# HydrogenSulfate/LFT

Measured on AMD Instinct MI355X. Metric: LF patches/sec (5x5 angRes, 32x32 LR, 4xSR), higher is better.
Workload: dtype bf16; 1 GPU; LFT 5x5 angRes 4xSR inference, batch=4 per GPU, 32x32 LR patches; global_batch=4, parallelism=dp1 (independent shards), streams_per_gpu=1, hip_graph=True, steps_in_flight=2

## Files before the change

### lft_amd/csrc/lft_api.hip

```cpp
#include "../../include/lft_hip.h"
#include "../../include/lft_hip_test.h"
#include <hip/hip_runtime.h>
#include <stdint.h>

#include <cstdarg>
#include <cstdio>
#include <cmath>
#include <set>
#include <string>
#include <algorithm>
#include <type_traits>
#include <utility>
#include <vector>

#ifndef LFT_TU
#define LFT_TU 0
#endif

namespace {
#include "lft_kernels_a.cuh"
#include "lft_kernels_b.cuh"
#include "lft_metrics.cuh"
#include "lft_train.cuh"
}
// ... 9 lines not shown

int fail(int code, const char* fmt, ...) {
    va_list ap;
    va_start(ap, fmt);
    vsnprintf(g_err, sizeof(g_err), fmt, ap);
    va_end(ap);
    return code;
}

#define LFT_HIP_OK(expr)                                                                     \
    do {                                                                                     \
        hipError_t e_ = (expr);                                                              \
        if (e_ != hipSuccess) return fail((int)e_, "%s: %s", #expr, hipGetErrorString(e_));   \
    } while (0)
struct Profiler {
    bool on = false;
    hipStream_t st = nullptr;
    std::vector<hipEvent_t> ev;
    std::vector<const char*> names;
};
thread_local Profiler g_prof;
inline const char* prof_name(const char* plain, const char* fmt, ...) {
    if (!g_prof.on) return plain;
    static thread_local std::set<std::string> names;
    char buf[96];
    va_list ap;
    va_start(ap, fmt);
    vsnprintf(buf, sizeof(buf), fmt, ap);
    va_end(ap);
    return names.insert(buf).first->c_str();
}
inline void prof_mark(const char* name) {
    if (!g_prof.on) return;
    hipEvent_t e;
    if (hipEventCreate(&e) != hipSuccess) return;
    (void)hipEventRecord(e, g_prof.st);
    g_prof.ev.push_back(e);
    g_prof.names.push_back(name);
}

#define LFT_LAUNCH_OK(name)                                                                  \
    do {                                                                                     \
        hipError_t e_ = hipGetLastError();                                                   \
        if (e_ != hipSuccess) return fail((int)e_, "launch %s: %s", name, hipGetErrorString(e_)); \
        prof_mark(name);                                                                     \
    } while (0)

constexpr int kLayers = 4;

template <auto... Vs, typename V, typename F> int dispatch(V v, F&& f) {
    int rc = 0;
    if (((v == Vs && ((rc = f(std::integral_constant<decltype(Vs), Vs>{})), true)) || ...)) return rc;
    return fail(LFT_ERR_ARG, "internal: no kernel variant for %d", (int)v);
}
template <int V> using int_c = std::integral_constant<int, V>;
template <typename F> int by_prec(int prec, F&& f) {
    if (prec == LFT_PREC_F32) return f(float{});
    if (prec == LFT_PREC_BF16) return f(bf16_t{});
    return f(f16_t{});
}
inline size_t align256(size_t x) { return (x + 255) & ~(size_t)255; }

struct Dims {
    int B, A, V, h, w, hw, s, gp, gt, nchunk;
    long long ntok;
};

int make_dims(int B, int A, int h, int w, int s, int prec, Dims* d) {
    if (prec != LFT_PREC_F32 && prec != LFT_PREC_BF16 && prec != LFT_PREC_F16)
        return fail(LFT_ERR_ARG, "prec must be LFT_PREC_F32, LFT_PREC_BF16 or LFT_PREC_F16, got %d", prec);
    if (B < 1 || A < 1 || h < 1 || w < 1) return fail(LFT_ERR_SHAPE, "B, A, h, w must be positive (B=%d A=%d h=%d w=%d)", B, A, h, w);
    if (s != 2 && s != 4) return fail(LFT_ERR_SHAPE, "scale factor must be 2 or 4, got %d", s);
    if (A * A > 128) return fail(LFT_ERR_UNSUPPORTED, "angRes %d (A*A=%d views > 128) is not implemented in this build", A, A * A);
    if ((long long)B * A * A * h * w > (1LL << 27)) return fail(LFT_ERR_SHAPE, "too many tokens");
    d->B = B; d->A = A; d->V = A * A; d->h = h; d->w = w; d->hw = h * w; d->s = s;
    d->gp = (s + 2) * (s + 2); d->gt = (d->gp + 31) / 32; d->nchunk = 2 * s * s;
    d->ntok = (long long)B * d->V * d->hw;
    return 0;
}

constexpr int kFragsConv = 72, kFragsAng = 64, kFragsSpa1 = 240, kFragsSpa1NoQ = 208, kFragsSpa2 = 176;
inline int frags_up(const Dims& d) { return d.nchunk * (4 + 2 * d.gt); }

struct PackedLayout {
    size_t conv0_w, ln_ang[kLayers], ln_spa[kLayers], ang_pe, petok[kLayers], spa_pe_img;
    size_t s_conv[3], s_ang[kLayers], s_spa1[kLayers], s_spa2[kLayers], s_up, total;
};

PackedLayout packed_layout(const Dims& d, int prec) {
    const size_t esz = prec == LFT_PREC_F32 ? 4 : 2, fragb = 64 * 8 * esz;
    PackedLayout L;
    size_t o = 0;
    auto take = [&](size_t bytes) { size_t r = o; o = align256(o + bytes); return r; };
    L.conv0_w = take(576 * 4);
    for (int l = 0; l < kLayers; ++l) { L.ln_ang[l] = take(256 * 4); L.ln_spa[l] = take(512 * 4); }
    L.ang_pe = take((size_t)((d.V + 31) / 32) * 2048 * 4);
    for (int l = 0; l < kLayers; ++l) L.petok[l] = take((size_t)((d.hw + 32 * kNwSpa1 - 1) / (32 * kNwSpa1)) * kNwSpa1 * 4096 * esz);
    L.spa_pe_img = take((size_t)d.hw * 64 * esz);
    for (int i = 0; i < 3; ++i) L.s_conv[i] = take(kFragsConv * fragb);
    for (int l = 0; l < kLayers; ++l) {
        L.s_ang[l] = take(kFragsAng * fragb);
        L.s_spa1[l] = take(kFragsSpa1 * fragb);
        L.s_spa2[l] = take(kFragsSpa2 * fragb);
    }
    L.s_up = take((size_t)frags_up(d) * fragb);
    L.total = o;
    return L;
}

struct WorkLayout {
    size_t x0, feat, xa, xb, tok, q, k, v, o, g, status, total;
};
WorkLayout work_layout(const Dims& d, int prec) {
    const size_t esz = prec == LFT_PREC_F32 ? 4 : 2;
    WorkLayout W;
    size_t o = 0;
    auto take = [&](size_t bytes) { size_t r = o; o = align256(o + bytes); return r; };
    const size_t n = (size_t)d.ntok;
    W.x0 = take(n * 64 * esz); W.feat = take(n * 64 * esz); W.xa = take(n * 64 * esz); W.xb = take(n * 64 * esz);
    W.tok = take(n * 128 * esz); W.q = take(n * 128 * esz); W.k = take(n * 128 * esz); W.v = take(n * 128 * esz);
    W.o = take(n * 128 * esz);
    W.g = take(n * d.gp * 4);
    W.status = take(256);
    W.total = o;
    return W;
}

template <typename T> size_t lds_conv64(int w) { return WRing<T, kConv64Chunk, kNwConv>::LDS_BYTES + ConvIn<T, kNwConv>::bytes(w) + kNwConv * TileIO<2, T>::BYTES + kConvZeroRow; }
constexpr size_t kLdsParams = 1024;
template <typename T, int CH = kSpaChunk> size_t lds_spa1(int w) {
    return WRing<T, CH, kNwSpa1>::LDS_BYTES + std::max<size_t>(ConvIn<T, kNwSpa1>::bytes(w), (size_t)kNwSpa1 * TileIO<4, T>::BYTES) + kLdsParams + kConvZeroRow;
}
template <typename T> size_t lds_spa2() { return WRing<T, kSpaChunk, kNwSpa2>::LDS_BYTES + kLdsParams + kNwSpa2 * TileIO<4, T>::BYTES; }
template <typename T> size_t lds_up() { return WRing<T, kUpChunk, kNwUp>::LDS_BYTES + kNwUp * TileIO<2, T>::BYTES; }
template <typename T> size_t lds_ang() { return (size_t)kFragsAng * 1024 * FragInfo<T>::PIECES + kLdsParams + 4 * TileIO<2, T>::BYTES; }
constexpr size_t kMaxLds = 160 * 1024;
template <typename K> int allow_lds(K kernel, size_t bytes, const char* name) {
    if (bytes > kMaxLds) return fail(LFT_ERR_SHAPE, "%s needs %zu B of LDS (> 160 KiB): view width too large for this build", name, bytes);
    if (bytes <= 64 * 1024) return 0;
    struct Done { int dev; const void* fn; size_t bytes; };
    static thread_local std::vector<Done> done;
    const void* fn = reinterpret_cast<const void*>(kernel);
    int dev = 0;
    LFT_HIP_OK(hipGetDevice(&dev));
    for (const auto& d : done)
        if (d.dev == dev && d.fn == fn && d.bytes >= bytes) return 0;
    LFT_HIP_OK(hipFuncSetAttribute(fn, hipFuncAttributeMaxDynamicSharedMemorySize, (int)bytes));
    done.push_back(Done{dev, fn, bytes});
    return 0;
}

template <typename P> P* at(const void* base, size_t off) { return reinterpret_cast<P*>(const_cast<char*>(static_cast<const char*>(base)) + off); }
inline unsigned blocks_for(long long items, int per_block) { return (unsigned)((items + per_block - 1) / per_block); }

PackOp lin_op(const float* src, int row0, int nrows, int ld, int k0, int ksteps, int kmap, float scale, int kmul = 1, int kadd = 0) {
    PackOp p{};
    p.src = src; p.kind = 0; p.row0 = row0; p.nrows = nrows; p.ntiles = (nrows + 31) / 32; p.ld = ld;
    p.kmul = kmul; p.kadd = kadd; p.k0 = k0; p.ksteps = ksteps; p.kmap = kmap; p.scale = scale; p.s = 0; p.frag0 = 0;
    return p;
}
void conv_ops(std::vector<PackOp>& v, const float* w, int nout) {
    for (int tap = 0; tap < 9; ++tap)
        for (int ks = 0; ks < 4; ++ks) v.push_back(lin_op(w, 0, nout, 576, 16 * ks, 1, 0, 1.0f, 9, tap));
}

template <typename T>
int run_pack(std::vector<PackOp>& ops, T* dst, int expect_frags, hipStream_t st) {
    int total = 0;
    size_t i = 0;
    while (i < ops.size()) {
        PackArgs a{};
        int nf = 0;
        while (i < ops.size() && a.nops < LFT_PACK_MAXOPS) {
            a.op[a.nops] = ops[i];
            a.op[a.nops].frag0 = nf;
            nf += ops[i].ntiles * ops[i].ksteps;
            ++a.nops; ++i;
        }
        k_pack<T><<<nf, 64, 0, st>>>(a, dst + (size_t)total * 512);
        LFT_LAUNCH_OK("k_pack");
        total += nf;
    }
    if (total != expect_frags) return fail(LFT_ERR_ARG, "internal: stream has %d fragments, expected %d", total, expect_frags);
    return 0;
}

template <typename T> bool tok_lane_major(const Dims& d) {
    return d.hw % (32 * kNwSpa1) == 0 && (sizeof(T) == 4 || d.w % 32 == 0);
}
template <typename T, bool PE_ONLY>
int launch_spa1(unsigned nwg, const T* in, const T* ws, const float* ln, const T* petok, T* tok, T* q, T* k, T* v, T* pe_out,
                int nimg, const Dims& d, hipStream_t st, unsigned* status) {
    const size_t l16 = lds_spa1<T, 16>(d.w), l8 = lds_spa1<T, 8>(d.w);
    const size_t share = kMaxLds / kSpaOcc;
    const bool use8 = (l16 > share && l8 <= share) || l16 > kMaxLds;
    const bool lm = !PE_ONLY && tok_lane_major<T>(d);
    return dispatch<8, 16>(use8 ? 8 : 16, [&](auto CH) {
        return dispatch<true, false>(lm, [&](auto LM) {
            constexpr bool WQ = !(LM && sizeof(T) == 2);
            const size_t lds = CH == 8 ? l8 : l16;
            if (int rc = allow_lds(k_spa1<T, PE_ONLY, CH, LM, WQ>, lds, "k_spa1")) return rc;
            k_spa1<T, PE_ONLY, CH, LM, WQ><<<nwg, 64 * kNwSpa1, lds, st>>>(in, ws, ln, petok, tok, q, k, v, pe_out, nimg, d.h, d.w, status);
            return 0;
        });
    });
}

template <typename T>
int pack_impl(const float* const* P, void* packed, const Dims& d, int prec, hipStream_t st) {
    const PackedLayout L = packed_layout(d, prec);
    const float kAngScale = 0.35355339059327373f * LFT_LOG2E;
    const float kSpaScale = 0.25f * LFT_LOG2E;
    int rc;
    k_copy_f32<<<3, 256, 0, st>>>(P[0], at<float>(packed, L.conv0_w), 576);
    LFT_LAUNCH_OK("k_copy_f32");
    for (int i = 0; i < 3; ++i) {
        std::vector<PackOp> ops;
        conv_ops(ops, P[1 + i], 64);
        if ((rc = run_pack<T>(ops, at<T>(packed, L.s_conv[i]), kFragsConv, st))) return rc;
    }
    k_pe_tables<T><<<blocks_for(std::max<long long>((long long)((d.V + 31) / 32) * 2048, (long long)d.hw * 64), 256), 256, 0, st>>>(
        at<float>(packed, L.ang_pe), at<T>(packed, L.spa_pe_img), d.V, d.h, d.w);
    LFT_LAUNCH_OK("k_pe_tables");
    for (int l = 0; l < kLayers; ++l) {
        const float* const* q = P + 4 + 18 * l;
        float* lnS = at<float>(packed, L.ln_spa[l]);
        float* lnA = at<float>(packed, L.ln_ang[l]);
        const int srcS[4] = {1, 2, 5, 6}, srcA[4] = {10, 11, 14, 15};
        for (int j = 0; j < 4; ++j) {
            k_copy_f32<<<1, 256, 0, st>>>(q[srcS[j]], lnS + 128 * j, 128);
            k_copy_f32<<<1, 256, 0, st>>>(q[srcA[j]], lnA + 64 * j, 64);
        }
        LFT_LAUNCH_OK("k_copy_f32");
        {
            std::vector<PackOp> ops;
            ops.push_back(lin_op(q[12], 0, 64, 64, 0, 4, 1, kAngScale));
            ops.push_back(lin_op(q[12], 64, 64, 64, 0, 4, 1, 1.0f));
            ops.push_back(lin_op(q[12], 128, 64, 64, 0, 4, 1, 1.0f));
            ops.push_back(lin_op(q[13], 0, 64, 64, 0, 4, 1, 1.0f));
            ops.push_back(lin_op(q[16], 0, 128, 64, 0, 4, 1, 1.0f));
            ops.push_back(lin_op(q[17], 0, 64, 128, 0, 8, 1, 1.0f));
            if ((rc = run_pack<T>(ops, at<T>(packed, L.s_ang[l]), kFragsAng, st))) return rc;
        }
        {
            std::vector<PackOp> ops;
            conv_ops(ops, q[0], 128);
            ops.push_back(lin_op(q[3], 256, 128, 128, 0, 8, 1, 1.0f));
            ops.push_back(lin_op(q[3], 128, 128, 128, 0, 8, 1, 1.0f));
            ops.push_back(lin_op(q[3], 0, 128, 128, 0, 8, 1, kSpaScale));
            if ((rc = run_pack<T>(ops, at<T>(packed, L.s_spa1[l]), kFragsSpa1, st))) return rc;
        }
        {
            std::vector<PackOp> ops;
            ops.push_back(lin_op(q[4], 0, 128, 128, 0, 8, (sizeof(T) == 2 && tok_lane_major<T>(d)) ? 1 : 0, 1.0f));
            for (int c = 0; c < 4; ++c) {
                ops.push_back(lin_op(q[7], 64 * c, 64, 128, 0, 8, 1, 1.0f));
                ops.push_back(lin_op(q[8], 0, 128, 256, 64 * c, 4, 1, 1.0f));
            }
            ops.push_back(lin_op(q[9], 0, 64, 128, 0, 8, 1, 1.0f));
            if ((rc = run_pack<T>(ops, at<T>(packed, L.s_spa2[l]), kFragsSpa2, st))) return rc;
        }
        if ((rc = launch_spa1<T, true>((unsigned)((d.hw + 32 * kNwSpa1 - 1) / (32 * kNwSpa1)), at<T>(packed, L.spa_pe_img), at<T>(packed, L.s_spa1[l]), nullptr, nullptr,
                                       nullptr, nullptr, nullptr, nullptr, at<T>(packed, L.petok[l]), 1, d, st, nullptr))) return rc;
        LFT_LAUNCH_OK("k_spa1<pe>");
    }
    {
        std::vector<PackOp> ops;
        for (int c = 0; c < d.nchunk; ++c) {
            ops.push_back(lin_op(P[76], 32 * c, 32, 64, 0, 4, 1, 1.0f));
            PackOp m = lin_op(P[77], 0, d.gp, 0, 32 * c, 2, 1, 1.0f);
            m.kind = 1; m.s = d.s; m.ntiles = d.gt;
            ops.push_back(m);
        }
        if ((rc = run_pack<T>(ops, at<T>(packed, L.s_up), frags_up(d), st))) return rc;
    }
    return 0;
}

void launch_assemble(const float* lr, const float* g, float* out, int B, int A, int h, int w, int s, hipStream_t st, int gld = 0, unsigned* status = nullptr) {
    const dim3 tg((unsigned)((A * w + 7) / 8) * (unsigned)((A * h + 7) / 8) * (unsigned)B);
    if (!gld) gld = (s + 2) * (s + 2);
    if (s == 2) k_assemble_t<2><<<tg, 256, 0, st>>>(lr, g, out, B, A, h, w, gld, status);
    else k_assemble_t<4><<<tg, 256, 0, st>>>(lr, g, out, B, A, h, w, gld, status);
}

template <typename T>
int init_features(const void* packed, const PackedLayout& L, const float* lr, T* x0, T* ta, T* tb, T* feat, const Dims& d, hipStream_t st) {
    const int nimg = d.B * d.V, nwg = nimg * ((d.hw + 32 * kNwConv - 1) / (32 * kNwConv));
    const size_t lds = lds_conv64<T>(d.w);
    int rc;
    if ((rc = allow_lds(k_conv64<T, false>, lds, "k_conv64"))) return rc;
    if ((rc = allow_lds(k_conv64<T, true>, lds, "k_conv64"))) return rc;
    k_conv0<T><<<dim3((unsigned)((d.hw + kConv0Tok - 1) / kConv0Tok), (unsigned)nimg), 256, 0, st>>>(lr, at<float>(packed, L.conv0_w), x0, d.B, d.A, d.h, d.w);
    LFT_LAUNCH_OK("k_conv0");
    k_conv64<T, false><<<nwg, 64 * kNwConv, lds, st>>>(x0, ta, nullptr, at<T>(packed, L.s_conv[0]), nimg, d.h, d.w);
    LFT_LAUNCH_OK("k_conv64");
    k_conv64<T, false><<<nwg, 64 * kNwConv, lds, st>>>(ta, tb, nullptr, at<T>(packed, L.s_conv[1]), nimg, d.h, d.w);
    LFT_LAUNCH_OK("k_conv64");
    k_conv64<T, true><<<nwg, 64 * kNwConv, lds, st>>>(tb, feat, x0, at<T>(packed, L.s_conv[2]), nimg, d.h, d.w);
    LFT_LAUNCH_OK("k_conv64");
    return 0;
}
template <typename T, int CT, int LL>
int ang_multi(const void* packed, const PackedLayout& L, int l, const T* in, T* out, const Dims& d, hipStream_t st, unsigned* status) {
    constexpr bool WLDS = sizeof(T) == 2;
    constexpr int NG = (sizeof(T) == 2 && CT <= 3) ? 2 : 1;
    constexpr size_t FB = 1024 * FragInfo<T>::PIECES;
    const size_t lds = (WLDS ? 64 * FB : 0) + 1024 + (size_t)NG * CT * 8 * FB + (size_t)NG * CT * TileIO<2, T>::BYTES;
    const int npix = d.B * d.hw;
    int rc;
    const unsigned grid = std::min<unsigned>(blocks_for(npix, NG), 256u * (unsigned)std::max<size_t>(1, kMaxLds / lds));
    if ((rc = allow_lds(k_ang_multi<T, CT, WLDS, NG, LL>, lds, "k_ang_multi"))) return rc;
    k_ang_multi<T, CT, WLDS, NG, LL><<<grid, 64 * CT * NG, lds, st>>>(in, out, at<T>(packed, L.s_ang[l]), at<float>(packed, L.ln_ang[l]),
                                                                     at<float>(packed, L.ang_pe), d.V, d.hw, npix, status);
    LFT_LAUNCH_OK("k_ang");
    return 0;
}
template <typename T>
int ang_block(const void* packed, const PackedLayout& L, int l, const T* in, T* out, const Dims& d, hipStream_t st, unsigned* status = nullptr) {
    auto multi = [&](auto CT, auto LL) { return ang_multi<T, CT, LL>(packed, L, l, in, out, d, st, status); };
    if (d.V > 100) return multi(int_c<4>{}, int_c<13>{});
    if (d.V > 96) return multi(int_c<4>{}, int_c<9>{});
    if (d.V > 64) return multi(int_c<3>{}, int_c<9>{});
    if (d.V == 64) return multi(int_c<2>{}, int_c<16>{});
    if (d.V > 32) return multi(int_c<2>{}, int_c<9>{});
    const int npix = d.B * d.hw;
    const size_t lds = lds_ang<T>();
    int rc;
    const unsigned grid = std::min<unsigned>(blocks_for(npix, 4), 256u * (unsigned)std::max<size_t>(1, kMaxLds / lds));
    if ((rc = allow_lds(k_ang<T, 13>, lds, "k_ang"))) return rc;
    k_ang<T, 13><<<grid, 256, lds, st>>>(in, out, at<T>(packed, L.s_ang[l]), at<float>(packed, L.ln_ang[l]),
                                         at<float>(packed, L.ang_pe), d.V, d.hw, npix, status);
    LFT_LAUNCH_OK("k_ang");
    return 0;
}
template <typename T>
int spa_part_a(const void* packed, const PackedLayout& L, int l, const T* in, void* ws, const WorkLayout& W, const Dims& d, hipStream_t st) {
    const int nimg = d.B * d.V, nwg = nimg * ((d.hw + 32 * kNwSpa1 - 1) / (32 * kNwSpa1));
    int rc;
    if ((rc = launch_spa1<T, false>((unsigned)nwg, in, at<T>(packed, L.s_spa1[l]), at<float>(packed, L.ln_spa[l]), at<T>(packed, L.petok[l]),
                                    at<T>(ws, W.tok), at<T>(ws, W.q), at<T>(ws, W.k), at<T>(ws, W.v), nullptr, nimg, d, st, at<unsigned>(ws, W.status)))) return rc;
    LFT_LAUNCH_OK("k_spa1");
    return 0;
}
template <typename F> int with_tail_variant(bool skip, bool tok_lm, bool out_lm, F&& launch) {
    if (out_lm) {
        if (!(skip && tok_lm)) return fail(LFT_ERR_ARG, "internal: lane-major output needs the skip variant and lane-major tokens");
        return launch(std::true_type{}, std::true_type{}, std::true_type{});
    }
    return dispatch<true, false>(skip, [&](auto SK) {
        return dispatch<true, false>(tok_lm, [&](auto LM) { return launch(SK, LM, std::false_type{}); });
    });
}
template <typename T>
int spa_part_b(const void* packed, const PackedLayout& L, int l, const T* skip, T* out, void* ws, const WorkLayout& W,
               const Dims& d, hipStream_t st, bool out_lm = false) {
    const int nimg = d.B * d.V;
    T *tok = at<T>(ws, W.tok), *q = at<T>(ws, W.q), *k = at<T>(ws, W.k), *v = at<T>(ws, W.v), *o = at<T>(ws, W.o);
    const float* ln = at<float>(packed, L.ln_spa[l]);
    const bool lm = tok_lane_major<T>(d);
    int rc;
    if constexpr (sizeof(T) == 2) {
        const unsigned ntile = (unsigned)(nimg * ((d.h + kAttTY - 1) / kAttTY) * ((d.w + kAttTX - 1) / kAttTX));
        if ((rc = with_tail_variant(skip, lm, out_lm, [&](auto SK, auto LM, auto YL) {
                 if (int r = allow_lds(k_spa_b<T, SK, LM, YL>, kSpaBLds, "k_spa_b")) return r;
                 k_spa_b<T, SK, LM, YL><<<ntile, 256, kSpaBLds, st>>>(tok, q, k, v, at<T>(packed, L.s_spa2[l]), ln, skip, out, d.h, d.w,
                                                                      at<unsigned>(ws, W.status), at<T>(packed, L.s_spa1[l]) + (size_t)kFragsSpa1NoQ * 512,
                                                                      at<T>(packed, L.petok[l]));
                 return 0;
             }))) return rc;
        LFT_LAUNCH_OK("k_spa_b");
        return 0;
    } else {
        const unsigned tiles = (unsigned)(((d.w + kWaTX - 1) / kWaTX) * ((d.h + kWaTY - 1) / kWaTY) * nimg);
        if ((rc = allow_lds(k_win_attn_lds<0, true>, kWaLds, "k_win_attn_lds"))) return rc;
        k_win_attn_lds<0, true><<<dim3(tiles, 4), 256, kWaLds, st>>>(reinterpret_cast<const float*>(q), reinterpret_cast<const float*>(k),
                                                                     reinterpret_cast<const float*>(v), reinterpret_cast<float*>(o),
                                                                     nullptr, nullptr, nullptr, nullptr, nullptr, d.h, d.w, 128);
        LFT_LAUNCH_OK("k_spa_attn");
        const unsigned nb = blocks_for(d.ntok, 32 * kNwSpa2);
        if ((rc = with_tail_variant(skip, lm, out_lm, [&](auto SK, auto LM, auto YL) {
                 if (int r = allow_lds(k_spa2<T, SK, LM, YL>, lds_spa2<T>(), "k_spa2")) return r;
                 k_spa2<T, SK, LM, YL><<<nb, 64 * kNwSpa2, lds_spa2<T>(), st>>>(tok, o, at<T>(packed, L.s_spa2[l]), ln, skip, out, d.ntok, at<unsigned>(ws, W.status));
                 return 0;
             }))) return rc;
        LFT_LAUNCH_OK("k_spa2");
        return 0;
    }
}
template <typename T>
int spa_block(const void* packed, const PackedLayout& L, int l, const T* in, const T* skip, T* out, void* ws, const WorkLayout& W,
              const Dims& d, hipStream_t st, bool out_lm = false) {
    int rc;
    if ((rc = spa_part_a<T>(packed, L, l, in, ws, W, d, st))) return rc;
    return spa_part_b<T>(packed, L, l, skip, out, ws, W, d, st, out_lm);
}
template <typename T>
int upsample(const void* packed, const PackedLayout& L, const T* body, const float* lr, float* out, void* ws, const WorkLayout& W,
             const Dims& d, hipStream_t st, bool in_lm = false) {
    float* g = at<float>(ws, W.g);
    const unsigned nb = blocks_for(d.ntok, 32 * kNwUp);
    int rc = dispatch<1, 2>(d.gt, [&](auto GT) {
        return dispatch<true, false>(in_lm, [&](auto LM) {
            if (int r = allow_lds(k_up<T, GT, LM>, lds_up<T>(), "k_up")) return r;
            k_up<T, GT, LM><<<nb, 64 * kNwUp, lds_up<T>(), st>>>(body, at<T>(packed, L.s_up), g, d.ntok, d.nchunk, d.gp);
            return 0;
        });
    });
    if (rc) return rc;
    LFT_LAUNCH_OK("k_up");
    launch_assemble(lr, g, out, d.B, d.A, d.h, d.w, d.s, st, 0, at<unsigned>(ws, W.status));
    LFT_LAUNCH_OK("k_assemble");
    return 0;
}

template <typename T>
int forward_impl(const void* packed, const float* lr, float* out, void* ws, const Dims& d, int prec, hipStream_t st) {
    const PackedLayout L = packed_layout(d, prec);
    const WorkLayout W = work_layout(d, prec);
    T *x0 = at<T>(ws, W.x0), *feat = at<T>(ws, W.feat), *xa = at<T>(ws, W.xa), *xb = at<T>(ws, W.xb);
    int rc;
    if ((rc = init_features<T>(packed, L, lr, x0, xa, xb, feat, d, st))) return rc;
    const T* cur = feat;
    for (int l = 0; l < kLayers; ++l) {
        if ((rc = ang_block<T>(packed, L, l, cur, xa, d, st, at<unsigned>(ws, W.status)))) return rc;
        const bool last = l == kLayers - 1;
        if ((rc = spa_block<T>(packed, L, l, xa, last ? feat : nullptr, xb, ws, W, d, st, last && tok_lane_major<T>(d)))) return rc;
        cur = xb;
    }
    return upsample<T>(packed, L, xb, lr, out, ws, W, d, st, tok_lane_major<T>(d));
}

template <typename T>
int kernel_time_impl(const char* name, const void* packed, void* ws, const Dims& d, int prec, int reps, hipStream_t st, float* ms_out) {
    const PackedLayout L = packed_layout(d, prec);
    const WorkLayout W = work_layout(d, prec);
    T *x0 = at<T>(ws, W.x0), *feat = at<T>(ws, W.feat), *xa = at<T>(ws, W.xa), *xb = at<T>(ws, W.xb);
    const std::string k(name);
    auto once = [&]() -> int {
        if (k == "k_ang") return ang_block<T>(packed, L, 1, xb, xa, d, st, at<unsigned>(ws, W.status));
        if (k == "k_spa1") return spa_part_a<T>(packed, L, 1, xa, ws, W, d, st);
        if (k == "k_spa_b" || k == "k_spa_attn+k_spa2") return spa_part_b<T>(packed, L, 1, nullptr, xb, ws, W, d, st);
        if (k == "k_conv64") {
            const int nimg = d.B * d.V, nwg = nimg * ((d.hw + 32 * kNwConv - 1) / (32 * kNwConv));
            const size_t lds = lds_conv64<T>(d.w);
            int rc;
            if ((rc = allow_lds(k_conv64<T, false>, lds, "k_conv64"))) return rc;
            k_conv64<T, false><<<nwg, 64 * kNwConv, lds, st>>>(x0, feat, nullptr, at<T>(packed, L.s_conv[0]), nimg, d.h, d.w);
            LFT_LAUNCH_OK("k_conv64");
            return 0;
        }
// ... 427 lines not shown
```

### lft_amd/csrc/lft_kernels_b.cuh

```cuda
#pragma once
#include "lft_common.cuh"
#include "lft_kernels_a.cuh"

constexpr int kUpChunk = 8;
constexpr int kSpaChunk = 16;
constexpr int kSpaOcc = 2;
constexpr int kNwSpa1 = 4, kNwSpa2 = 4, kNwUp = 8;
template <typename T, bool PE_ONLY, int CH = kSpaChunk, bool TOKLM = false, bool WITH_Q = true, int NW = kNwSpa1>
__global__ __launch_bounds__(64 * NW, kSpaOcc) void k_spa1(const T* __restrict__ X, const T* __restrict__ ws,
                                              const float* __restrict__ ln, const T* __restrict__ petok,
                                              T* __restrict__ TOK, T* __restrict__ Q, T* __restrict__ K, T* __restrict__ Vv,
                                              T* __restrict__ pe_out, int nimg, int h, int w, unsigned* __restrict__ status) {
    extern __shared__ __attribute__((aligned(16))) char smem[];
    const int lane = threadIdx.x & 63, r = lane & 31, hh = lane >> 5, wave = threadIdx.x >> 6;
    constexpr int TT = 32 * NW;
    const int hw = h * w, tpi = (hw + TT - 1) / TT;
    const int bid = xcd_tile(blockIdx.x, gridDim.x);
    const int im = bid / tpi, p0 = (bid % tpi) * TT;
    const int tl = wave * 32 + r, p = p0 + tl;
    const bool ok = p < hw;
    LFT_STAMP(0);
    typename RawPiece<T>::type pe_raw[16];
    if (!PE_ONLY) load_lane_major_raw<4, T>(petok + (size_t)((p0 >> 5) + wave) * 4096, lane, pe_raw);
    char* lds_in = smem + WRing<T, CH, NW>::LDS_BYTES;
// ... 62 lines not shown
            zero_acc<2>(a);
            linear_ring<2, 8, T>(ring, nf, a);
            if constexpr (QKVLM) store_tile_lm<2, T>(Q + lm_off + half * 2048, lane, a);
            else store_tile<2, T, 128>(Q + tile_off + 64 * half, nvalid, lane, a, scr);
        }
    }
    LFT_STAMP(11);
    publish_status(status, bad);
}

constexpr int kAttTY = 4, kAttTX = 32, kAttHR = kAttTY + 4, kAttHC = kAttTX + 4;
LFT_DEV int att_swz(int row, int col) { return (row & 1) | (((col >> 2) & 1) << 1); }
typedef short s16x4 __attribute__((ext_vector_type(4)));

template <typename T, bool SKIP, bool TOKLM = false, bool YLM = false, int NW = kNwSpa2>
__global__ __launch_bounds__(64 * NW, kSpaOcc) void k_spa2(const T* __restrict__ TOK, const T* __restrict__ O, const T* __restrict__ ws,
                                              const float* __restrict__ ln, const T* __restrict__ skip, T* __restrict__ Y,
                                              long long ntok, unsigned* __restrict__ status) {
    extern __shared__ __attribute__((aligned(16))) char smem[];
    const int lane = threadIdx.x & 63, r = lane & 31, hh = lane >> 5;
    const int wave = threadIdx.x >> 6;
    const long long t0 = ((long long)blockIdx.x * NW + wave) * 32;
    const int nvalid = (int)max(0LL, min(32LL, ntok - t0));
    const long long tb = min(t0, ntok - 1);
    char* scr = smem + WRing<T, kSpaChunk, NW>::LDS_BYTES + 1024 + wave * TileIO<4, T>::BYTES;
    WRing<T, kSpaChunk, NW> ring;
    LFT_STAMP(16);
    ring.init(ws, smem, 176);
    f32x16 t[4], n[4];
    if constexpr (TOKLM) load_tile_lm<4, T>(TOK + tb * 128, lane, t);
    else load_tile<4, T>(TOK + tb * 128, nvalid, lane, t, scr);
    Frag<T> f[8];
    load_tile_frags<8, T>(O + tb * 128, nvalid, lane, f, scr);
    f32x16 sk[2];
    if (SKIP) load_tile<2, T>(skip + tb * 64, nvalid, lane, sk, scr);
    float* lds_ln = reinterpret_cast<float*>(smem + WRing<T, kSpaChunk, NW>::LDS_BYTES);
    params_store(lds_ln, 256, params_load(ln + 256, 256));
    LFT_STAMP(17);
    linear_ring<4, 8, T>(ring, f, t);
    LFT_STAMP(18);
#pragma unroll
    for (int nt = 0; nt < 4; ++nt) n[nt] = t[nt];
    unsigned bad = 0;
    layernorm_acc<4>(n, lds_ln, lds_ln + 128, hh, bad);
    acc_frags<4, T>(n, f);
    LFT_STAMP(19);
#pragma unroll
    for (int c = 0; c < 4; ++c) {
        f32x16 hid[2];
        zero_acc<2>(hid);
        linear_ring<2, 8, T>(ring, f, hid);
        Frag<T> hf[4];
        acc_frags_relu<2>(hid, hf);
        linear_ring<4, 4, T>(ring, hf, t);
    }
    LFT_STAMP(20);
    acc_frags<4, T>(t, f);
    f32x16 y[2];
    zero_acc<2>(y);
    linear_ring<2, 8, T>(ring, f, y);
    if (SKIP) {
#pragma unroll
        for (int nt = 0; nt < 2; ++nt) y[nt] += sk[nt];
    }
    LFT_STAMP(21);
    if constexpr (YLM) store_tile_lm<2, T>(Y + tb * 64, lane, y);
    else store_tile<2, T>(Y + tb * 64, nvalid, lane, y, scr);
    LFT_STAMP(22);
    publish_status(status, bad);
}

constexpr int kSpaBChunk = 8;
constexpr int kAdTile = kAttHR * kAttHC * 64;
constexpr int kAdPerWave = 2 * kAdTile / 1024 / 4;
static_assert(2 * kAdTile == 4 * kAdPerWave * 1024, "the K and V tiles must split into whole pieces over 4 waves");
constexpr int kSpaBLds = 4 * kAdTile + 2048;
constexpr int kSpaBSlotsA = (2 * kAdTile) / (kSpaBChunk * 1024);
constexpr int kSpaBSlotsB = 2;
constexpr int kSpaBSlots = kSpaBSlotsA + kSpaBSlotsB;
constexpr int kSpaBScratchOfs = 16384;
static_assert(kSpaBScratchOfs + 4 * TileIO<4, bf16_t>::BYTES <= 2 * kAdTile, "scratch must fit buffer B");
static_assert(kSpaBSlotsB * kSpaBChunk * 1024 <= kSpaBScratchOfs, "the ring slots in buffer B must end before the scratch");

template <typename T> LFT_DEV void q_load_async(const T* p0, const T* p1, raw16& a, raw16& b) {
    asm volatile("global_load_dwordx4 %0, %2, off\n\tglobal_load_dwordx4 %1, %3, off" : "=&v"(a), "=&v"(b) : "v"(p0), "v"(p1) : "memory");
}
LFT_DEV void ld16_async(const void* p, raw16& d) { asm volatile("global_load_dwordx4 %0, %1, off" : "=v"(d) : "v"(p) : "memory"); }
template <int OFS> LFT_DEV void ld16_async_ofs(const void* p, raw16& d) {
    static_assert(OFS >= 0 && OFS < 4096, "global_load immediate offset");
    asm volatile("global_load_dwordx4 %0, %1, off offset:%2" : "=v"(d) : "v"(p), "n"(OFS) : "memory");
}
LFT_DEV void ld16_async_x8(const char* p, raw16 (&d)[8]) {
    const char* p2 = p + 4096;
    ld16_async_ofs<0>(p, d[0]); ld16_async_ofs<1024>(p, d[1]); ld16_async_ofs<2048>(p, d[2]); ld16_async_ofs<3072>(p, d[3]);
    ld16_async_ofs<0>(p2, d[4]); ld16_async_ofs<1024>(p2, d[5]); ld16_async_ofs<2048>(p2, d[6]); ld16_async_ofs<3072>(p2, d[7]);
}
template <int N> LFT_DEV void wait_vm_8(raw16 (&r)[8]) {
    asm volatile("s_waitcnt vmcnt(%8)" : "+v"(r[0]), "+v"(r[1]), "+v"(r[2]), "+v"(r[3]), "+v"(r[4]), "+v"(r[5]), "+v"(r[6]), "+v"(r[7]) : "n"(N) : "memory");
    __builtin_amdgcn_sched_barrier(0);
}
template <int N> LFT_DEV void wait_vm_only() {
    asm volatile("s_waitcnt vmcnt(%0)" :: "n"(N) : "memory");
    __builtin_amdgcn_sched_barrier(0);
}
template <int N> LFT_DEV void wait_vm_q(raw16& a, raw16& b) {
    asm volatile("s_waitcnt vmcnt(%2)" : "+v"(a), "+v"(b) : "n"(N) : "memory");
    __builtin_amdgcn_sched_barrier(0);
}

template <typename T> LFT_DEV void q_head_pair(const raw16 (&wr)[8], const Frag<T> (&nf)[8], Frag<T>& q0, Frag<T>& q1) {
    f32x16 q;
#pragma unroll
    for (int i = 0; i < 16; ++i) q[i] = 0.0f;
#pragma unroll
    for (int ks = 0; ks < 8; ++ks) {
        Frag<T> wf;
        wf.v = __builtin_bit_cast(typename H16<T>::v8, wr[ks]);
        mma(wf, nf[ks], q);
    }
    q0 = acc_to_frag(q, 0, T());
    q1 = acc_to_frag(q, 1, T());
}

template <typename T, bool SKIP, bool TOKLM = false, bool YLM = false>
__global__ __launch_bounds__(256, 2) void k_spa_b(const T* __restrict__ TOK, const T* __restrict__ Q, const T* __restrict__ K,
                                                  const T* __restrict__ Vv, const T* __restrict__ ws, const float* __restrict__ ln,
                                                  const T* __restrict__ skip, T* __restrict__ Y, int h, int w, unsigned* __restrict__ status,
                                                  const T* __restrict__ wq, const T* __restrict__ petok) {
    static_assert(sizeof(T) == 2, "k_spa_b is the 16-bit (bf16 / f16) part B; fp32 uses k_win_attn_lds + k_spa2");
    typedef typename H16<T>::v8 V8;
    using Ring = WRingPipe<T, kSpaBChunk, 4, kSpaBSlots, 176>;
    extern __shared__ __attribute__((aligned(16))) char smem[];
    char* const bufA = smem;
    char* const bufB = smem + 2 * kAdTile;
    float* lds_ln = reinterpret_cast<float*>(smem + 4 * kAdTile);
    const int tiles_x = (w + kAttTX - 1) / kAttTX, tiles_y = (h + kAttTY - 1) / kAttTY;
    const int bid = xcd_tile(blockIdx.x, gridDim.x);
    const int tx = bid % tiles_x, ty = (bid / tiles_x) % tiles_y, im = bid / (tiles_x * tiles_y);
    const int lane = threadIdx.x & 63, r = lane & 31, hh = lane >> 5;
    const int wave = __builtin_amdgcn_readfirstlane(threadIdx.x >> 6);
    const int y0 = ty * kAttTY, x0 = tx * kAttTX, bxl = 8 * wave;
    const long long img0 = (long long)im * h * w;
    LFT_STAMP(16);
    const int qpx = 4 * (r >> 4) + (r & 3), qpy = (r >> 2) & 3;
    const int qy = y0 + qpy, qx = x0 + bxl + qpx;
    const long long qtok = img0 + min(qy, h - 1) * w + min(qx, w - 1);
    const T* qptr = TOKLM ? Q + (img0 + (long long)min(qy, h - 1) * w + x0) * 128 + (32 * hh + bxl + qpx) * 8
                               : Q + qtok * 128 + 8 * hh;
    constexpr int kQHead = TOKLM ? 512 : 16, kQPair = 2 * kQHead;
    int dofs[kAdPerWave];
    {
        const int s0 = (wave & 1) * kAdPerWave * 16 + (lane >> 2), piece = lane & 3;
        int row = s0 / kAttHC, col = s0 % kAttHC;
#pragma unroll
        for (int i = 0; i < kAdPerWave; ++i) {
            const int gy = min(max(y0 - 2 + row, 0), h - 1), gx = min(max(x0 - 2 + col, 0), w - 1);
            const int tk = gy * w + gx;
            const int pq = piece ^ att_swz(row, col);
            const int pconst = TOKLM ? ((pq >> 1) * 512 + (pq & 1) * 256) * 2 : pq * 16;
            dofs[i] = (TOKLM ? ((tk & ~31) << 8) + ((tk & 31) << 4) : tk * 256) + pconst;
            col += 16;
            if (col >= kAttHC) { col -= kAttHC; row += 1; }
        }
    }
    constexpr int kDmaPair = TOKLM ? 2048 : 64;
    const char* const dsrc = reinterpret_cast<const char*>((wave < 2 ? K : Vv) + img0 * 128);
    const int ddst = (wave < 2 ? 0 : kAdTile) + (wave & 1) * kAdPerWave * 1024;
    auto stage = [&](int hg, char* buf) {
        LFT_DMA_NOTE("DMA", kNoteKV, hg & 1);
#pragma unroll
        for (int i = 0; i < kAdPerWave; ++i) glds16_asm(dsrc + dofs[i] + hg * kDmaPair, buf + ddst + i * 1024);
    };
    const int g4 = lane >> 4, qi = lane & 15;
    f32x4 bias[2][4];
    int kb[2], vb[2];
    auto setup_tiles = [&]() __attribute__((always_inline)) {
    {
        const int wy0 = max(0, qy - 2), wy1 = min(h, qy + 3), cy0 = y0 - 2;
        const int ya = min(max(wy0 - cy0, 0), 8), yb = min(max(wy1 - cy0, 0), 8);
        const unsigned ymask = ((1u << yb) - 1u) & ~((1u << ya) - 1u);
        const int gy = g4 >> 1, gx4 = 4 * (g4 & 1);
#pragma unroll
        for (int b = 0; b < 2; ++b) {
            const int bqx = x0 + bxl + 4 * b + (lane & 3), cx0 = x0 + bxl + 4 * b - 2;
            const int wx0 = max(0, bqx - 2), wx1 = min(min(h, bqx + 3), w);
            const int xa = min(max(wx0 - cx0, 0), 8), xb = min(max(wx1 - cx0, 0), 8);
            const unsigned xs = (((1u << xb) - 1u) & ~((1u << xa) - 1u)) >> gx4;
#pragma unroll
            for (int t = 0; t < 4; ++t) {
                const unsigned inval = ~(xs & (unsigned)__builtin_amdgcn_sbfe((int)ymask, 2 * t + gy, 1));
#pragma unroll
                for (int e = 0; e < 4; ++e)
                    bias[b][t][e] = __builtin_bit_cast(float, (unsigned)__builtin_amdgcn_sbfe((int)inval, e, 1) & 0xff800000u);
            }
        }
    }
    {
        const int ktok = ((qi >> 3) * kAttHC + bxl + (qi & 7)) * 64, ks0 = (qi >> 3) & 1, ks1 = (qi >> 2) & 1;
        const int vtok = ((g4 >> 1) * kAttHC + bxl + 4 * (g4 & 1) + (qi >> 2)) * 64, vs0 = (g4 >> 1) & 1, vs1 = g4 & 1, vp = qi & 3;
#pragma unroll
        for (int x = 0; x < 2; ++x) {
            kb[x] = ktok + 32 * (x ^ ks1) + 16 * ((g4 >> 1) ^ ks0) + 8 * (g4 & 1);
            vb[x] = kAdTile + vtok + 32 * (x ^ vs1) + 16 * ((vp >> 1) ^ vs0) + 8 * (vp & 1);
        }
    }
    };
    unsigned bad = 0;
    Frag<T> qfr[8];
    raw16 tokr[8];
    raw16 lnv;
    if constexpr (TOKLM) {
        raw16 lnv1, per[8], wqa[8], wqb[8];
        const int ty_ = min(qy, h - 1);
        const int lane_piece = (32 * hh + bxl + qpx) * 8;
        const char* tsrc = reinterpret_cast<const char*>(TOK + (img0 + (long long)ty_ * w + x0) * 128 + lane_piece);
        const char* psrc = reinterpret_cast<const char*>(petok + ((long long)ty_ * w + x0) * 128 + lane_piece);
        const char* wsrc = reinterpret_cast<const char*>(wq) + lane * 16;
        const int pi = min((int)threadIdx.x * 4, 252);
        ld16_async(ln + pi, lnv1);
        ld16_async(ln + 256 + pi, lnv);
        ld16_async_x8(tsrc, tokr);
        ld16_async_x8(psrc, per);
        ld16_async_x8(wsrc, wqa);
        ld16_async_x8(wsrc + 8 * 1024, wqb);
        stage(0, bufA);
        stage(1, bufB);
        wait_vm_8<16 + 2 * kAdPerWave>(tokr);
        wait_vm_8<16 + 2 * kAdPerWave>(per);
        asm volatile("" : "+v"(lnv), "+v"(lnv1));
        params_store(lds_ln, 256, lnv);
        params_store(lds_ln + 256, 256, lnv1);
        wg_barrier_keep_vm();
        f32x16 n[4];
#pragma unroll
        for (int kidx = 0; kidx < 8; ++kidx) {
            const V8 vt = __builtin_bit_cast(V8, tokr[kidx]), vp = __builtin_bit_cast(V8, per[kidx]);
#pragma unroll
            for (int j = 0; j < 8; ++j) n[kidx >> 1][8 * (kidx & 1) + j] = (float)vt[j] + (float)vp[j];
        }
        layernorm_acc<4, true>(n, lds_ln + 256, lds_ln + 256 + 128, hh, bad);
        Frag<T> nf[8];
        acc_frags<4, T>(n, nf);
        wait_vm_8<8 + 2 * kAdPerWave>(wqa);
        q_head_pair<T>(wqa, nf, qfr[0], qfr[1]);
        ld16_async_x8(wsrc + 16 * 1024, wqa);
        wait_vm_8<2 * kAdPerWave + 8>(wqb);
        q_head_pair<T>(wqb, nf, qfr[2], qfr[3]);
        ld16_async_x8(wsrc + 24 * 1024, wqb);
        wait_vm_8<8>(wqa);
        q_head_pair<T>(wqa, nf, qfr[4], qfr[5]);
        wait_vm_8<0>(wqb);
        q_head_pair<T>(wqb, nf, qfr[6], qfr[7]);
#pragma unroll
        for (int hd = 0; hd < 8; ++hd) {
            raw16 f = __builtin_bit_cast(raw16, qfr[hd].v);
            frag_to_blocks(f);
            qfr[hd].v = __builtin_bit_cast(V8, f);
        }
    } else {
        lnv = params_load(ln + 256, 256);
        stage(0, bufA);
        stage(1, bufB);
    }
    Ring ring;
    ring.setup(ws, smem, kSpaBSlotsA, 2 * kAdTile - kSpaBSlotsA * kSpaBChunk * 1024);
    BlkRows rows;
    rows.nrow = max(0, min(4, h - y0)); rows.ncol = max(0, min(8, w - (x0 + bxl)));
    if (rows.ncol == 0) rows.nrow = 0;
    const long long tok0 = img0 + (long long)min(y0, h - 1) * w + min(x0 + bxl, w - 1);
    setup_tiles();
    LFT_STAMP(17);
    raw16 qa, qb;
    if constexpr (!TOKLM) q_load_async(qptr, qptr + kQHead, qa, qb);
    Frag<T> of[8];
    __builtin_amdgcn_s_setprio(3);
#pragma unroll
    for (int hg = 0; hg < 4; ++hg) {
        char* const buf = (hg & 1) ? bufB : bufA;
        if constexpr (TOKLM) {
            if (hg == 0) wait_vm_only<0>();
            else if (hg < 3) wait_vm_only<kAdPerWave>();
            else wait_vm_only<kSpaBSlotsA * Ring::PIECES_PER_WAVE>();
        } else {
            if (hg == 0) { wait_vm_q<0>(qa, qb); params_store(lds_ln, 256, lnv); }
            else if (hg < 3) wait_vm_q<kAdPerWave>(qa, qb);
            else wait_vm_q<kSpaBSlotsA * Ring::PIECES_PER_WAVE>(qa, qb);
        }
        wg_barrier_keep_vm();
        LFT_NOTE_ASM_("USE", kNoteKV, hg & 1);
        LFT_STAMP(18 + 2 * hg);
        raw16 qf[2];
        if constexpr (TOKLM) { qf[0] = __builtin_bit_cast(raw16, qfr[2 * hg].v); qf[1] = __builtin_bit_cast(raw16, qfr[2 * hg + 1].v); }
        else { qf[0] = qa; qf[1] = qb; frag_to_blocks(qf[0]); frag_to_blocks(qf[1]); }
#pragma unroll
        for (int hl = 0; hl < 2; ++hl) {
            f32x4 S[2][4];
            float m0 = -INFINITY, m1 = -INFINITY;
#pragma unroll
            for (int b = 0; b < 2; ++b)
#pragma unroll
                for (int t = 0; t < 4; ++t) {
                    const u32x2 kf = *reinterpret_cast<const u32x2*>(buf + kb[hl ^ b] + (2 * t * kAttHC + 4 * b) * 64);
                    S[b][t] = mfma16k16(kf, u32x2{qf[hl][2 * b], qf[hl][2 * b + 1]}, bias[b][t], T());
#pragma unroll
                    for (int e = 0; e < 4; ++e) { if (b == 0) m0 = fmaxf(m0, S[b][t][e]); else m1 = fmaxf(m1, S[b][t][e]); }
                }
            xrow_combine2(m0, m1, [](float a, float b) { return max_fast(a, b); });
// ... 372 lines not shown
```

Before: 9759 patches/s.

## Precompute spa_b DMA offsets and window bias bits into a packed table

```diff
diff --git a/lft_amd/csrc/lft_api.hip b/lft_amd/csrc/lft_api.hip
--- a/lft_amd/csrc/lft_api.hip
+++ b/lft_amd/csrc/lft_api.hip
@@ -115,8 +115,14 @@
 constexpr int kFragsConv = 72, kFragsAng = 64, kFragsSpa1 = 240, kFragsSpa1NoQ = 208, kFragsSpa2 = 176;
 inline int frags_up(const Dims& d) { return d.nchunk * (4 + 2 * d.gt); }
 
+template <typename T> bool tok_lane_major(const Dims& d) {
+    return d.hw % (32 * kNwSpa1) == 0 && (sizeof(T) == 4 || d.w % 32 == 0);
+}
+inline bool spa_b_tables(const Dims& d, int prec) { return prec != LFT_PREC_F32 && tok_lane_major<bf16_t>(d); }
+inline int spa_b_tiles(const Dims& d) { return ((d.h + kAttTY - 1) / kAttTY) * ((d.w + kAttTX - 1) / kAttTX); }
+
 struct PackedLayout {
-    size_t conv0_w, ln_ang[kLayers], ln_spa[kLayers], ang_pe, petok[kLayers], spa_pe_img;
+    size_t conv0_w, ln_ang[kLayers], ln_spa[kLayers], ang_pe, petok[kLayers], spa_pe_img, spa_geo;
     size_t s_conv[3], s_ang[kLayers], s_spa1[kLayers], s_spa2[kLayers], s_up, total;
 };
 
@@ -130,6 +136,7 @@
     L.ang_pe = take((size_t)((d.V + 31) / 32) * 2048 * 4);
     for (int l = 0; l < kLayers; ++l) L.petok[l] = take((size_t)((d.hw + 32 * kNwSpa1 - 1) / (32 * kNwSpa1)) * kNwSpa1 * 4096 * esz);
     L.spa_pe_img = take((size_t)d.hw * 64 * esz);
+    L.spa_geo = take(spa_b_tables(d, prec) ? (size_t)spa_b_tiles(d) * 4 * kSpaGeoWave : 0);
     for (int i = 0; i < 3; ++i) L.s_conv[i] = take(kFragsConv * fragb);
     for (int l = 0; l < kLayers; ++l) {
         L.s_ang[l] = take(kFragsAng * fragb);
@@ -218,9 +225,6 @@
     return 0;
 }
 
-template <typename T> bool tok_lane_major(const Dims& d) {
-    return d.hw % (32 * kNwSpa1) == 0 && (sizeof(T) == 4 || d.w % 32 == 0);
-}
 template <typename T, bool PE_ONLY>
 int launch_spa1(unsigned nwg, const T* in, const T* ws, const float* ln, const T* petok, T* tok, T* q, T* k, T* v, T* pe_out,
                 int nimg, const Dims& d, hipStream_t st, unsigned* status) {
@@ -255,6 +259,10 @@
     k_pe_tables<T><<<blocks_for(std::max<long long>((long long)((d.V + 31) / 32) * 2048, (long long)d.hw * 64), 256), 256, 0, st>>>(
         at<float>(packed, L.ang_pe), at<T>(packed, L.spa_pe_img), d.V, d.h, d.w);
     LFT_LAUNCH_OK("k_pe_tables");
+    if (spa_b_tables(d, prec)) {
+        k_spa_b_geo<<<(unsigned)spa_b_tiles(d), 256, 0, st>>>(at<char>(packed, L.spa_geo), d.h, d.w, (d.w + kAttTX - 1) / kAttTX);
+        LFT_LAUNCH_OK("k_spa_b_geo");
+    }
     for (int l = 0; l < kLayers; ++l) {
         const float* const* q = P + 4 + 18 * l;
         float* lnS = at<float>(packed, L.ln_spa[l]);
@@ -399,7 +407,7 @@
                  if (int r = allow_lds(k_spa_b<T, SK, LM, YL>, kSpaBLds, "k_spa_b")) return r;
                  k_spa_b<T, SK, LM, YL><<<ntile, 256, kSpaBLds, st>>>(tok, q, k, v, at<T>(packed, L.s_spa2[l]), ln, skip, out, d.h, d.w,
                                                                       at<unsigned>(ws, W.status), at<T>(packed, L.s_spa1[l]) + (size_t)kFragsSpa1NoQ * 512,
-                                                                      at<T>(packed, L.petok[l]));
+                                                                      at<T>(packed, L.petok[l]), at<char>(packed, L.spa_geo));
                  return 0;
              }))) return rc;
         LFT_LAUNCH_OK("k_spa_b");
diff --git a/lft_amd/csrc/lft_kernels_b.cuh b/lft_amd/csrc/lft_kernels_b.cuh
--- a/lft_amd/csrc/lft_kernels_b.cuh
+++ b/lft_amd/csrc/lft_kernels_b.cuh
@@ -168,10 +168,72 @@
 static_assert(kSpaBScratchOfs + 4 * TileIO<4, bf16_t>::BYTES <= 2 * kAdTile, "scratch must fit buffer B");
 static_assert(kSpaBSlotsB * kSpaBChunk * 1024 <= kSpaBScratchOfs, "the ring slots in buffer B must end before the scratch");
 
+template <bool TOKLM> LFT_DEV void spa_b_dofs(int wave, int lane, int y0, int x0, int h, int w, int (&dofs)[kAdPerWave]) {
+    const int s0 = (wave & 1) * kAdPerWave * 16 + (lane >> 2), piece = lane & 3;
+    int row = s0 / kAttHC, col = s0 % kAttHC;
+#pragma unroll
+    for (int i = 0; i < kAdPerWave; ++i) {
+        const int gy = min(max(y0 - 2 + row, 0), h - 1), gx = min(max(x0 - 2 + col, 0), w - 1);
+        const int tk = gy * w + gx;
+        const int pq = piece ^ att_swz(row, col);
+        const int pconst = TOKLM ? ((pq >> 1) * 512 + (pq & 1) * 256) * 2 : pq * 16;
+        dofs[i] = (TOKLM ? ((tk & ~31) << 8) + ((tk & 31) << 4) : tk * 256) + pconst;
+        col += 16;
+        if (col >= kAttHC) { col -= kAttHC; row += 1; }
+    }
+}
+struct SpaBWindow { unsigned ymask, xs[2]; int gy; };
+LFT_DEV SpaBWindow spa_b_window(int wave, int lane, int y0, int x0, int h, int w) {
+    SpaBWindow m;
+    const int r = lane & 31, g4 = lane >> 4, bxl = 8 * wave;
+    const int qy = y0 + ((r >> 2) & 3);
+    const int wy0 = max(0, qy - 2), wy1 = min(h, qy + 3), cy0 = y0 - 2;
+    const int ya = min(max(wy0 - cy0, 0), 8), yb = min(max(wy1 - cy0, 0), 8);
+    m.ymask = ((1u << yb) - 1u) & ~((1u << ya) - 1u);
+    m.gy = g4 >> 1;
+    const int gx4 = 4 * (g4 & 1);
+#pragma unroll
+    for (int b = 0; b < 2; ++b) {
+        const int bqx = x0 + bxl + 4 * b + (lane & 3), cx0 = x0 + bxl + 4 * b - 2;
+        const int wx0 = max(0, bqx - 2), wx1 = min(min(h, bqx + 3), w);
+        const int xa = min(max(wx0 - cx0, 0), 8), xb = min(max(wx1 - cx0, 0), 8);
+        m.xs[b] = (((1u << xb) - 1u) & ~((1u << xa) - 1u)) >> gx4;
+    }
+    return m;
+}
+LFT_DEV unsigned spa_b_inval(const SpaBWindow& m, int b, int t) {
+    return ~(m.xs[b] & (unsigned)__builtin_amdgcn_sbfe((int)m.ymask, 2 * t + m.gy, 1));
+}
+constexpr int kSpaGeoWave = 2560;
+LFT_DEV unsigned spa_b_bias_bits(const SpaBWindow& m) {
+    unsigned bits = 0;
+#pragma unroll
+    for (int b = 0; b < 2; ++b)
+#pragma unroll
+        for (int t = 0; t < 4; ++t) bits |= (spa_b_inval(m, b, t) & 15u) << (16 * b + 4 * t);
+    return bits;
+}
+__global__ __launch_bounds__(256) void k_spa_b_geo(char* __restrict__ geo, int h, int w, int tiles_x) {
+    const int tile = blockIdx.x, lane = threadIdx.x & 63, wave = threadIdx.x >> 6;
+    const int y0 = (tile / tiles_x) * kAttTY, x0 = (tile % tiles_x) * kAttTX;
+    int dofs[kAdPerWave];
+    spa_b_dofs<true>(wave, lane, y0, x0, h, w, dofs);
+    const unsigned bits = spa_b_bias_bits(spa_b_window(wave, lane, y0, x0, h, w));
+    char* base = geo + (size_t)(tile * 4 + wave) * kSpaGeoWave;
+    unsigned* p0 = reinterpret_cast<unsigned*>(base + lane * 16);
+    unsigned* p1 = reinterpret_cast<unsigned*>(base + 1024 + lane * 16);
+    unsigned* p2 = reinterpret_cast<unsigned*>(base + 2048 + lane * 8);
+#pragma unroll
+    for (int i = 0; i < 4; ++i) { p0[i] = (unsigned)dofs[i]; p1[i] = (unsigned)dofs[4 + i]; }
+    p2[0] = (unsigned)dofs[8];
+    p2[1] = bits;
+}
+
 template <typename T> LFT_DEV void q_load_async(const T* p0, const T* p1, raw16& a, raw16& b) {
     asm volatile("global_load_dwordx4 %0, %2, off\n\tglobal_load_dwordx4 %1, %3, off" : "=&v"(a), "=&v"(b) : "v"(p0), "v"(p1) : "memory");
 }
 LFT_DEV void ld16_async(const void* p, raw16& d) { asm volatile("global_load_dwordx4 %0, %1, off" : "=v"(d) : "v"(p) : "memory"); }
+LFT_DEV void ld8_async(const void* p, u32x2& d) { asm volatile("global_load_dwordx2 %0, %1, off" : "=v"(d) : "v"(p) : "memory"); }
 template <int OFS> LFT_DEV void ld16_async_ofs(const void* p, raw16& d) {
     static_assert(OFS >= 0 && OFS < 4096, "global_load immediate offset");
     asm volatile("global_load_dwordx4 %0, %1, off offset:%2" : "=v"(d) : "v"(p), "n"(OFS) : "memory");
@@ -212,7 +274,8 @@
 __global__ __launch_bounds__(256, 2) void k_spa_b(const T* __restrict__ TOK, const T* __restrict__ Q, const T* __restrict__ K,
                                                   const T* __restrict__ Vv, const T* __restrict__ ws, const float* __restrict__ ln,
                                                   const T* __restrict__ skip, T* __restrict__ Y, int h, int w, unsigned* __restrict__ status,
-                                                  const T* __restrict__ wq, const T* __restrict__ petok) {
+                                                  const T* __restrict__ wq, const T* __restrict__ petok,
+                                                  const char* __restrict__ geo) {
     static_assert(sizeof(T) == 2, "k_spa_b is the 16-bit (bf16 / f16) part B; fp32 uses k_win_attn_lds + k_spa2");
     typedef typename H16<T>::v8 V8;
     using Ring = WRingPipe<T, kSpaBChunk, 4, kSpaBSlots, 176>;
@@ -235,20 +298,7 @@
                                : Q + qtok * 128 + 8 * hh;
     constexpr int kQHead = TOKLM ? 512 : 16, kQPair = 2 * kQHead;
     int dofs[kAdPerWave];
-    {
-        const int s0 = (wave & 1) * kAdPerWave * 16 + (lane >> 2), piece = lane & 3;
-        int row = s0 / kAttHC, col = s0 % kAttHC;
-#pragma unroll
-        for (int i = 0; i < kAdPerWave; ++i) {
-            const int gy = min(max(y0 - 2 + row, 0), h - 1), gx = min(max(x0 - 2 + col, 0), w - 1);
-            const int tk = gy * w + gx;
-            const int pq = piece ^ att_swz(row, col);
-            const int pconst = TOKLM ? ((pq >> 1) * 512 + (pq & 1) * 256) * 2 : pq * 16;
-            dofs[i] = (TOKLM ? ((tk & ~31) << 8) + ((tk & 31) << 4) : tk * 256) + pconst;
-            col += 16;
-            if (col >= kAttHC) { col -= kAttHC; row += 1; }
-        }
-    }
+    if constexpr (!TOKLM) spa_b_dofs<false>(wave, lane, y0, x0, h, w, dofs);
     constexpr int kDmaPair = TOKLM ? 2048 : 64;
     const char* const dsrc = reinterpret_cast<const char*>((wave < 2 ? K : Vv) + img0 * 128);
     const int ddst = (wave < 2 ? 0 : kAdTile) + (wave & 1) * kAdPerWave * 1024;
@@ -260,26 +310,27 @@
     const int g4 = lane >> 4, qi = lane & 15;
     f32x4 bias[2][4];
     int kb[2], vb[2];
+    unsigned gbits = 0;
     auto setup_tiles = [&]() __attribute__((always_inline)) {
-    {
-        const int wy0 = max(0, qy - 2), wy1 = min(h, qy + 3), cy0 = y0 - 2;
-        const int ya = min(max(wy0 - cy0, 0), 8), yb = min(max(wy1 - cy0, 0), 8);
-        const unsigned ymask = ((1u << yb) - 1u) & ~((1u << ya) - 1u);
-        const int gy = g4 >> 1, gx4 = 4 * (g4 & 1);
-#pragma unroll
-        for (int b = 0; b < 2; ++b) {
-            const int bqx = x0 + bxl + 4 * b + (lane & 3), cx0 = x0 + bxl + 4 * b - 2;
-            const int wx0 = max(0, bqx - 2), wx1 = min(min(h, bqx + 3), w);
-            const int xa = min(max(wx0 - cx0, 0), 8), xb = min(max(wx1 - cx0, 0), 8);
-            const unsigned xs = (((1u << xb) - 1u) & ~((1u << xa) - 1u)) >> gx4;
+    if constexpr (TOKLM) {
+#pragma unroll
+        for (int b = 0; b < 2; ++b)
+#pragma unroll
+            for (int t = 0; t < 4; ++t)
+#pragma unroll
+                for (int e = 0; e < 4; ++e)
+                    bias[b][t][e] = __builtin_bit_cast(float, (unsigned)__builtin_amdgcn_sbfe((int)gbits, 16 * b + 4 * t + e, 1) & 0xff800000u);
+    } else {
+        const SpaBWindow m = spa_b_window(wave, lane, y0, x0, h, w);
+#pragma unroll
+        for (int b = 0; b < 2; ++b)
 #pragma unroll
             for (int t = 0; t < 4; ++t) {
-                const unsigned inval = ~(xs & (unsigned)__builtin_amdgcn_sbfe((int)ymask, 2 * t + gy, 1));
+                const unsigned inval = spa_b_inval(m, b, t);
 #pragma unroll
                 for (int e = 0; e < 4; ++e)
                     bias[b][t][e] = __builtin_bit_cast(float, (unsigned)__builtin_amdgcn_sbfe((int)inval, e, 1) & 0xff800000u);
             }
-        }
     }
     {
         const int ktok = ((qi >> 3) * kAttHC + bxl + (qi & 7)) * 64, ks0 = (qi >> 3) & 1, ks1 = (qi >> 2) & 1;
@@ -296,19 +347,30 @@
     raw16 tokr[8];
     raw16 lnv;
     if constexpr (TOKLM) {
-        raw16 lnv1, per[8], wqa[8], wqb[8];
+        raw16 lnv1, per[8], wqa[8], wqb[8], geo0, geo1;
+        u32x2 geo2;
         const int ty_ = min(qy, h - 1);
         const int lane_piece = (32 * hh + bxl + qpx) * 8;
         const char* tsrc = reinterpret_cast<const char*>(TOK + (img0 + (long long)ty_ * w + x0) * 128 + lane_piece);
         const char* psrc = reinterpret_cast<const char*>(petok + ((long long)ty_ * w + x0) * 128 + lane_piece);
         const char* wsrc = reinterpret_cast<const char*>(wq) + lane * 16;
         const int pi = min((int)threadIdx.x * 4, 252);
+        const char* gsrc = geo + (size_t)((ty * tiles_x + tx) * 4 + wave) * kSpaGeoWave;
+        ld16_async(gsrc + lane * 16, geo0);
+        ld16_async(gsrc + 1024 + lane * 16, geo1);
+        ld8_async(gsrc + 2048 + lane * 8, geo2);
         ld16_async(ln + pi, lnv1);
         ld16_async(ln + 256 + pi, lnv);
         ld16_async_x8(tsrc, tokr);
         ld16_async_x8(psrc, per);
         ld16_async_x8(wsrc, wqa);
         ld16_async_x8(wsrc + 8 * 1024, wqb);
+        asm volatile("s_waitcnt vmcnt(34)" : "+v"(geo0), "+v"(geo1), "+v"(geo2) :: "memory");
+        __builtin_amdgcn_sched_barrier(0);
+#pragma unroll
+        for (int i = 0; i < 4; ++i) { dofs[i] = (int)geo0[i]; dofs[4 + i] = (int)geo1[i]; }
+        dofs[8] = (int)geo2[0];
+        gbits = geo2[1];
         stage(0, bufA);
         stage(1, bufB);
         wait_vm_8<16 + 2 * kAdPerWave>(tokr);
```

Measured after the change: 9600 patches/s (median of 2 runs). 1.6% lower.
